# OwshenNetwork/owshen

Hardware: NVIDIA H100
Metric: groth16_withdraw_proofs_per_sec (higher is better)
Workload: dtype u256 (8x32-bit Montgomery limbs, integer)

## Files before the change

### bindings/rust/ffi.rs

```rust
#![allow(non_camel_case_types, dead_code)]
use std::os::raw::{c_char, c_void};

#[repr(C)] pub struct OgCtx { _private: [u8; 0] }
#[repr(C)] pub struct OgPk { _private: [u8; 0] }

pub const OG_OK: i32 = 0;
pub const OG_E_INVALID: i32 = -1;
pub const OG_E_ENCODING: i32 = -2;
pub const OG_E_NO_DEVICE: i32 = -3;
pub const OG_E_CUDA: i32 = -4;
pub const OG_E_NOMEM: i32 = -5;
pub const OG_E_VERIFY: i32 = -6;

extern "C" {
    pub fn og_abi_version() -> i32;
    pub fn og_strerror(code: i32) -> *const c_char;
    pub fn og_last_error(ctx: *const OgCtx) -> *const c_char;
    pub fn og_init(device: i32, out: *mut *mut OgCtx) -> i32;
    pub fn og_free(ctx: *mut OgCtx);
    pub fn og_sync(ctx: *mut OgCtx) -> i32;
    pub fn og_stream(ctx: *mut OgCtx, out_cuda_stream: *mut *mut c_void) -> i32;
    pub fn og_timer_start(ctx: *mut OgCtx) -> i32;
    pub fn og_timer_stop(ctx: *mut OgCtx, ms: *mut f32) -> i32;
    pub fn og_launch_count(ctx: *const OgCtx) -> u64;
// ... 91 lines not shown
    pub fn og_groth16_prove_labeled_association_dev(ctx: *mut OgCtx, pk: *const OgPk, d_tokens: *const u8, d_recipients: *const u8, d_withdrawn: *const u64, d_nullifiers: *const u8, d_secrets: *const u8, d_amounts: *const u64, d_labels: *const u32, d_siblings: *const u8, d_path_bits: *const u32, d_change_nullifiers: *const u8, d_change_secrets: *const u8, d_assoc_siblings: *const u8, d_assoc_path_bits: *const u32, batch: u32, d_rs: *const u8, d_proofs: *mut u8, d_public_out: *mut u8) -> i32;
    pub fn og_groth16_prove_owned_transfer(ctx: *mut OgCtx, pk: *const OgPk, roots: *const u8, tokens: *const u8, recipients: *const u8, in_spend_keys: *const u8, in_blindings: *const u8, in_amounts: *const u64, in_siblings: *const u8, in_path_bits: *const u32, out_owners: *const u8, out_blindings: *const u8, out_amounts: *const u64, batch: u32, rs: *const u8, proofs: *mut u8, public_out: *mut u8) -> i32;
    pub fn og_groth16_prove_owned_transfer_dev(ctx: *mut OgCtx, pk: *const OgPk, d_roots: *const u8, d_tokens: *const u8, d_recipients: *const u8, d_in_spend_keys: *const u8, d_in_blindings: *const u8, d_in_amounts: *const u64, d_in_siblings: *const u8, d_in_path_bits: *const u32, d_out_owners: *const u8, d_out_blindings: *const u8, d_out_amounts: *const u64, batch: u32, d_rs: *const u8, d_proofs: *mut u8, d_public_out: *mut u8) -> i32;
    pub fn og_groth16_h_evals(ctx: *mut OgCtx, pk: *const OgPk, witness: *const u8, out: *mut u8) -> i32;
    pub fn og_groth16_verify(vk: *const u8, vk_len: u64, public_inputs: *const u8, n_pub: u32, proof256: *const u8) -> i32;
    pub fn og_ptau_new(ctx: *mut OgCtx, log_max: u32, out: *mut u8, out_len: *mut u64) -> i32;
    pub fn og_ptau_contribute(ctx: *mut OgCtx, acc: *const u8, acc_len: u64, secrets96: *const u8, nonces96: *const u8, acc_out: *mut u8, acc_out_len: *mut u64, record_out: *mut u8, record_len: *mut u64) -> i32;
    pub fn og_ptau_verify(ctx: *mut OgCtx, prev: *const u8, prev_len: u64, next: *const u8, next_len: u64, record: *const u8, record_len: u64) -> i32;
    pub fn og_ptau_prepare(ctx: *mut OgCtx, acc: *const u8, acc_len: u64, n_constraints: u32, n_vars: u32, n_pub: u32, a_row_ptr: *const u32, a_col: *const u32, a_coeffs: *const u8, b_row_ptr: *const u32, b_col: *const u32, b_coeffs: *const u8, c_row_ptr: *const u32, c_col: *const u32, c_coeffs: *const u8, pk_out: *mut u8, pk_len: *mut u64, vk_out: *mut u8, vk_len: *mut u64) -> i32;
    pub fn og_ptau_prepare_withdraw(ctx: *mut OgCtx, acc: *const u8, acc_len: u64, depth: u32, pk_out: *mut u8, pk_len: *mut u64, vk_out: *mut u8, vk_len: *mut u64) -> i32;
    pub fn og_phase2_contribute(ctx: *mut OgCtx, pk: *const u8, pk_len: u64, vk: *const u8, vk_len: u64, delta32: *const u8, nonce32: *const u8, pk_out: *mut u8, pk_out_len: *mut u64, vk_out: *mut u8, vk_out_len: *mut u64, record_out: *mut u8, record_len: *mut u64) -> i32;
    pub fn og_phase2_verify(ctx: *mut OgCtx, pk_prev: *const u8, pk_prev_len: u64, vk_prev: *const u8, vk_prev_len: u64, pk_next: *const u8, pk_next_len: u64, vk_next: *const u8, vk_next_len: u64, record: *const u8, record_len: u64) -> i32;
    pub fn og_scale_points(ctx: *mut OgCtx, g2: i32, points: *const u8, scalars: *const u8, n: u64, per_point: i32, out: *mut u8) -> i32;
    pub fn og_intt_points(ctx: *mut OgCtx, g2: i32, points: *mut u8, log_m: u32) -> i32;
    pub fn og_msm_bucket_sums(ctx: *mut OgCtx, g2: i32, points: *const u8, n_points: u32, counts: *const u32, entries: *const u32, n_groups: u32, nb: u32, n_entries_max: u64, few_groups: i32, out_totals: *mut u8, out_buckets: *mut u8) -> i32;
    pub fn og_field_probe_raw(ctx: *mut OgCtx, unit: i32, op: i32, a: *const u8, b: *const u8, n: u64, out: *mut u8) -> i32;
}
```

### include/owshen_b200.h

```cpp
#ifndef OWSHEN_B200_H
#define OWSHEN_B200_H
#include <stdint.h>
#ifdef __cplusplus
extern "C" {
#endif

typedef struct og_ctx og_ctx;
typedef struct og_pk og_pk;

enum {
    OG_OK = 0,
    OG_E_INVALID = -1,
    OG_E_ENCODING = -2,
    OG_E_NO_DEVICE = -3,
    OG_E_CUDA = -4,
    OG_E_NOMEM = -5,
    OG_E_VERIFY = -6
};

int32_t og_abi_version(void);
const char* og_strerror(int32_t code);
const char* og_last_error(const og_ctx* ctx);

int32_t og_init(int32_t device, og_ctx** out);
// ... 260 lines not shown
int32_t og_ptau_prepare_withdraw(og_ctx* ctx, const uint8_t* acc, uint64_t acc_len, uint32_t depth, uint8_t* pk_out, uint64_t* pk_len,
                                 uint8_t* vk_out, uint64_t* vk_len);
int32_t og_phase2_contribute(og_ctx* ctx, const uint8_t* pk, uint64_t pk_len, const uint8_t* vk, uint64_t vk_len, const uint8_t* delta32,
                             const uint8_t* nonce32, uint8_t* pk_out, uint64_t* pk_out_len, uint8_t* vk_out, uint64_t* vk_out_len,
                             uint8_t* record_out, uint64_t* record_len);
int32_t og_phase2_verify(og_ctx* ctx, const uint8_t* pk_prev, uint64_t pk_prev_len, const uint8_t* vk_prev, uint64_t vk_prev_len,
                         const uint8_t* pk_next, uint64_t pk_next_len, const uint8_t* vk_next, uint64_t vk_next_len,
                         const uint8_t* record, uint64_t record_len);
int32_t og_scale_points(og_ctx* ctx, int32_t g2, const uint8_t* points, const uint8_t* scalars, uint64_t n, int32_t per_point,
                        uint8_t* out);
int32_t og_intt_points(og_ctx* ctx, int32_t g2, uint8_t* points, uint32_t log_m);

int32_t og_msm_bucket_sums(og_ctx* ctx, int32_t g2, const uint8_t* points, uint32_t n_points, const uint32_t* counts,
                           const uint32_t* entries, uint32_t n_groups, uint32_t nb, uint64_t n_entries_max, int32_t few_groups,
                           uint8_t* out_totals, uint8_t* out_buckets);
int32_t og_field_probe_raw(og_ctx* ctx, int32_t unit, int32_t op, const uint8_t* a, const uint8_t* b, uint64_t n, uint8_t* out);

#ifdef __cplusplus
}
#endif
#endif
```

### owshen_b200/api.py

```python
import array
import bisect
import ctypes as C
import os
import secrets as _rand
import subprocess

_HERE = os.path.dirname(os.path.abspath(__file__))
_LIB_PATH = os.environ.get("OWSHEN_B200_LIB") or os.path.join(_HERE, "libowshen_b200.so")
_lib = None

FR_MODULUS = 21888242871839275222246405745257275088548364400416034343698204186575808495617
PROOF_BYTES = 256

OG_OK, OG_E_INVALID, OG_E_VERIFY = 0, -1, -6

NOTE_SUBGROUP_ORDER = 2736030358979909402780800718157159386076813972158567259200215660948447373041
NOTE_NOT_OWNED, NOTE_MALFORMED = 0xFFFFFFFF, 0xFFFFFFFE
NOTE_RECORD_BYTES, NOTE_PLAINTEXT_BYTES = 160, 128


class OwshenB200Error(RuntimeError):
    def __init__(self, code, detail=""):
        self.code = code
        msg = lib().og_strerror(code).decode() if _lib is not None else str(code)
# ... 121 lines not shown
    "og_ptau_contribute": (C.c_int32, [C.c_void_p, C.c_void_p, C.c_uint64, C.c_void_p, C.c_void_p,
                                       C.c_void_p, C.POINTER(C.c_uint64), C.c_void_p, C.POINTER(C.c_uint64)]),
    "og_ptau_verify": (C.c_int32, [C.c_void_p, C.c_void_p, C.c_uint64, C.c_void_p, C.c_uint64, C.c_void_p, C.c_uint64]),
    "og_ptau_prepare": (C.c_int32, [C.c_void_p, C.c_void_p, C.c_uint64, C.c_uint32, C.c_uint32, C.c_uint32] + [C.c_void_p] * 9
                        + [C.c_void_p, C.POINTER(C.c_uint64), C.c_void_p, C.POINTER(C.c_uint64)]),
    "og_ptau_prepare_withdraw": (C.c_int32, [C.c_void_p, C.c_void_p, C.c_uint64, C.c_uint32,
                                             C.c_void_p, C.POINTER(C.c_uint64), C.c_void_p, C.POINTER(C.c_uint64)]),
    "og_phase2_contribute": (C.c_int32, [C.c_void_p, C.c_void_p, C.c_uint64, C.c_void_p, C.c_uint64, C.c_void_p, C.c_void_p,
                                         C.c_void_p, C.POINTER(C.c_uint64), C.c_void_p, C.POINTER(C.c_uint64),
                                         C.c_void_p, C.POINTER(C.c_uint64)]),
    "og_phase2_verify": (C.c_int32, [C.c_void_p] + [C.c_void_p, C.c_uint64] * 5),
    "og_scale_points": (C.c_int32, [C.c_void_p, C.c_int32, C.c_void_p, C.c_void_p, C.c_uint64, C.c_int32, C.c_void_p]),
    "og_intt_points": (C.c_int32, [C.c_void_p, C.c_int32, C.c_void_p, C.c_uint32]),
    "og_msm_bucket_sums": (C.c_int32, [C.c_void_p, C.c_int32, C.c_void_p, C.c_uint32, C.c_void_p, C.c_void_p, C.c_uint32, C.c_uint32,
                                       C.c_uint64, C.c_int32, C.c_void_p, C.c_void_p]),
    "og_field_probe_raw": (C.c_int32, [C.c_void_p, C.c_int32, C.c_int32, C.c_void_p, C.c_void_p, C.c_uint64, C.c_void_p]),
}
ABI_SYMBOLS = tuple(_SIGS)


def lib():
    global _lib
    if _lib is None:
        if not os.path.exists(_LIB_PATH):
            raise OSError(f"{_LIB_PATH} is missing: build it with owshen_b200.build_library() / "
                          "`make -C owshen_b200/csrc` -- there is no CPU fallback")
        L = C.CDLL(_LIB_PATH)
        for name, (res, args) in _SIGS.items():
            fn = getattr(L, name)
            fn.restype = res
# ... 227 lines not shown
            if not hasattr(xs, "astype"):
                return array.array("I", xs)
            a = array.array("I")
            a.frombytes(xs.astype("<u4").tobytes())
            return a
        cnt, ent = u32(counts), u32(entries)
        total = sum(cnt)
        _need(len(cnt) == n_groups * nb and len(ent) == total, "msm_bucket_sums: need n_groups * nb counts and sum(counts) entries")
        out = C.create_string_buffer(pb * n_groups)
        bk = C.create_string_buffer(pb * n_groups * nb) if buckets else None
        _check(lib().og_msm_bucket_sums(self._h, curve == "g2", points, len(points) // pb, C.c_void_p(cnt.buffer_info()[0]),
                                        C.c_void_p(ent.buffer_info()[0]) if total else None, n_groups, nb,
                                        total if n_entries_max is None else n_entries_max, int(few_groups), out, bk), self)
        return out.raw, (bk.raw if buckets else None)

    def mimc7_hash2(self, left: bytes, right: bytes) -> bytes:
        _need(len(left) % 32 == 0 and len(right) == len(left), "mimc7_hash2: left and right must be equally long multiples of 32 bytes")
        n = len(left) // 32
        out = C.create_string_buffer(32 * n)
        _check(lib().og_mimc7_hash2(self._h, left, right, n, out), self)
        return out.raw

    def merkle_paths(self, leaves: bytes, siblings: bytes, path_bits, depth: int) -> bytes:
        _need(0 <= depth <= 32 and len(leaves) % 32 == 0, "merkle_paths: depth must be <= 32 and leaves a multiple of 32 bytes")
        n = len(leaves) // 32
        _need(len(siblings) == 32 * n * depth and len(path_bits) == n, "merkle_paths: siblings must hold n*depth elements and path_bits n words")
        out = C.create_string_buffer(32 * n * (depth + 1))
        _check(lib().og_mimc7_merkle_paths(self._h, leaves, siblings, _bits_array(path_bits), n, depth, out), self)
        return out.raw

# ... 885 lines not shown
```

### owshen_b200/csrc/capi.cu

```cuda
#include <stdlib.h>
#include <new>
#include "common.cuh"
#include "groth16.cuh"
#include "mimc.cuh"
#include "msm.cuh"
#include "ntt.cuh"
#include "withdraw_circuit.hpp"

using namespace og;

void* og_ctx::slot(int id, size_t bytes) {
    if (bytes == 0) bytes = 32;
    if (slot_cap[id] >= bytes) return slot_ptr[id];
    cudaDeviceSynchronize();
    if (slot_ptr[id]) cudaFree(slot_ptr[id]);
    slot_ptr[id] = nullptr; slot_cap[id] = 0;
    size_t cap = bytes + bytes / 8;
    cudaError_t e = cudaMalloc(&slot_ptr[id], cap);
    if (e != cudaSuccess) {
        e = cudaMalloc(&slot_ptr[id], bytes);
        cap = bytes;
    }
    if (e != cudaSuccess) {
        snprintf(err, sizeof(err), "slot %d: cudaMalloc(%zu) failed: %s", id, bytes, cudaGetErrorString(e));
// ... 1457 lines not shown
    OG_SLOT(ctx, dtot, uint8_t, S_IO_E, pb * n_groups);
    uint8_t* dbk = nullptr;
    if (out_buckets) { dbk = (uint8_t*)ctx->slot(S_IO_F, pb * n_keys); if (!dbk) return OG_E_NOMEM; }
    OG_TRY(clear_flag(ctx));
    if (n_points) H2D(ctx, dp, points, pb * n_points);
    if (total) H2D(ctx, de, entries, 4 * total);
    H2D(ctx, dc, counts, 4ull * n_keys);
    H2D(ctx, doff, offsets.data(), 4ull * (n_keys + 1ull));
    if (g2) OG_TRY(msm_bucket_sums<Fq2>(ctx, dp, n_points, de, doff, dc, n_groups, nb, n_entries_max, few_groups != 0, dtot, dbk));
    else OG_TRY(msm_bucket_sums<Fq>(ctx, dp, n_points, de, doff, dc, n_groups, nb, n_entries_max, few_groups != 0, dtot, dbk));
    D2H(ctx, out_totals, dtot, pb * n_groups);
    if (out_buckets) D2H(ctx, out_buckets, dbk, pb * n_keys);
    return check_flag(ctx);
}

int32_t og_field_probe_raw(og_ctx* ctx, int32_t unit, int32_t op, const uint8_t* a, const uint8_t* b, uint64_t n, uint8_t* out) {
    OG_ENTER(ctx);
    const bool op_ok = unit ? (op >= 0 && op <= 7) : ((op >= 0 && op <= 3) || (op >= 8 && op <= 14));
    if (unit < 0 || unit > 1 || !op_ok || (n && (!a || !b || !out))) return OG_E_INVALID;
    if (n == 0) return OG_OK;
    const uint64_t eb = unit ? 64 : 32;
    OG_SLOT(ctx, da, uint8_t, S_IO_A, eb * n);
    OG_SLOT(ctx, db, uint8_t, S_IO_B, eb * n);
    OG_SLOT(ctx, dout, uint8_t, S_IO_C, eb * n);
    H2D(ctx, da, a, eb * n); H2D(ctx, db, b, eb * n);
    if (unit) OG_TRY(field_probe_raw<Fq2>(ctx, op, da, db, n, dout));
    else OG_TRY(field_probe_raw<Fq>(ctx, op, da, db, n, dout));
    D2H(ctx, out, dout, eb * n);
    OG_CUDA(ctx, cudaStreamSynchronize(ctx->stream));
    return OG_OK;
// ... 4 lines not shown
```

### owshen_b200/csrc/groth16.cu

```cuda
#include "groth16.cuh"
#include "mimc.cuh"
#include "msm.cuh"
#include "ntt.cuh"
#include "withdraw_circuit.hpp"
#include <stdlib.h>

namespace og {

__global__ void __launch_bounds__(128) k_extras(const uint8_t* __restrict__ rs, uint32_t batch, uint32_t n_vars, uint32_t w_stride,
                                                Fr* __restrict__ W, Fr* __restrict__ rs_m, int* flag) {
    uint32_t p = blockIdx.x * blockDim.x + threadIdx.x;
    if (p >= batch) return;
    Fr r = load_canonical<Fr>(rs + 64ull * p, flag);
    Fr s = load_canonical<Fr>(rs + 64ull * p + 32, flag);
    Fr* w = W + (size_t)p * w_stride;
    w[n_vars] = Fr::one();
    w[n_vars + 1] = r;
    rs_m[2 * p] = r;
    rs_m[2 * p + 1] = s;
}

__global__ void __launch_bounds__(128) k_witness_in(const uint8_t* __restrict__ in, uint32_t batch, uint32_t n_vars, uint32_t w_stride,
                                                    Fr* __restrict__ W, int* flag) {
    uint64_t t = (uint64_t)blockIdx.x * blockDim.x + threadIdx.x;
// ... 19 lines not shown
    if (j >= m) return;
    const Fr* w = W + (size_t)p * w_stride;
    Fr a = Fr::zero(), b = Fr::zero();
    if (j < n_constraints) {
        for (uint32_t k = A.row_ptr[j]; k < A.row_ptr[j + 1]; k++) a = a + A.val[k] * w[A.col[k]];
        for (uint32_t k = B.row_ptr[j]; k < B.row_ptr[j + 1]; k++) b = b + B.val[k] * w[B.col[k]];
    } else if (j <= n_constraints + n_pub) {
        a = w[j - n_constraints];
    }
    Fr* o = abc + (size_t)p * 3 * m;
    o[j] = a;
    o[m + j] = b;
    o[2 * m + j] = a * b;
}

__global__ void __launch_bounds__(128) k_pointwise(const Fr* __restrict__ abc, uint32_t log_m, uint32_t batch, Fr* __restrict__ csc,
                                                   uint32_t csc_stride, uint32_t off) {
    uint32_t m = 1u << log_m;
    uint32_t j = blockIdx.x * blockDim.x + threadIdx.x;
    uint32_t p = blockIdx.y;
    if (j >= m) return;
    const Fr* o = abc + (size_t)p * 3 * m;
    csc[(size_t)p * csc_stride + off + j] = o[j] * o[m + j] - o[2 * m + j];
}

__global__ void __launch_bounds__(128) k_compose(const Fr* __restrict__ W, uint32_t w_stride, const Fr* __restrict__ rs_m,
                                                 const uint32_t* __restrict__ supp, uint32_t n_supp, uint32_t n_vars, uint32_t n_pub,
                                                 uint32_t m, Fr* __restrict__ bsc, uint32_t bsc_stride, Fr* __restrict__ csc,
                                                 uint32_t csc_stride) {
    uint32_t t = blockIdx.x * blockDim.x + threadIdx.x;
    uint32_t p = blockIdx.y;
    const Fr* w = W + (size_t)p * w_stride;
    Fr* bs = bsc + (size_t)p * bsc_stride;
    Fr* cs = csc + (size_t)p * csc_stride;
    uint32_t n_priv = n_vars - n_pub - 1;
    Fr r = rs_m[2 * p], s = rs_m[2 * p + 1];
    if (t < n_priv) cs[t] = w[n_pub + 1 + t];
    if (t < n_supp) {
        Fr v = w[supp[t]];
        bs[t] = v;
        cs[n_priv + t] = r * v;
    }
    if (t == 0) {
        bs[n_supp] = Fr::one();
        bs[n_supp + 1] = s;
        cs[n_priv + n_supp + m] = r;
    }
}

__global__ void __launch_bounds__(32) k_assemble_g1(const G1XYZZ* __restrict__ totA, const G1XYZZ* __restrict__ totC,
                                                    const Fr* __restrict__ rs_m, uint32_t batch, uint8_t* __restrict__ proofs) {
    uint32_t p = blockIdx.x * blockDim.x + threadIdx.x;
    if (p >= batch) return;
    G1XYZZ a = totA[p];
    G1Affine A;
    xyzz_to_affine_ni(&A, &a);
    uint32_t s[8];
    rs_m[2 * p + 1].to_canonical(s);
    G1XYZZ acc = G1XYZZ::inf();
    for (int i = 255; i >= 0; i--) {
        xyzz_dbl_ni(&acc);
// ... 268 lines not shown
    b.sort_tiles = !s.tiles ? b.heavy : (uint32_t*)ctx->slot(S(S_PR_SORT_TILES, S_L1_SORT_TILES), s.tiles);
    if (!b.sort_stage || !b.sort_tiles) return OG_E_NOMEM;
    b.totC = b.totA + batch;
    b.totB = reinterpret_cast<G2XYZZ*>(b.totC + batch);
    return OG_OK;
}

template <class F>
static int32_t run_msm(og_ctx* ctx, const og_pk* pk, int which, ChunkBufs& b, uint32_t B, const Affine<F>* table, uint32_t n_pts,
                       const Fr* scalars, uint32_t stride, XYZZ<F>* totals) {
    DigitPlan plan;
    plan.scalars = reinterpret_cast<const uint32_t*>(scalars);
    plan.n = n_pts; plan.scalar_stride = stride; plan.n_problems = B;
    plan.c = pk->c[which]; plan.n_windows = pk->n_windows[which]; plan.nb = pk->nb[which];
    plan.key_stride_problem = 1; plan.key_stride_window = 0; plan.tidx_window_stride = n_pts;
    plan.montgomery = 1;
    uint32_t n_keys = B * pk->nb[which];
    OG_TRY(msm_sort_digits(ctx, plan, n_keys, b.counts, b.offsets, nullptr, b.sorted, b.sort_stage, b.sort_tiles));
    return msm_buckets(ctx, table, b.sorted, b.offsets, b.counts, B, pk->nb[which], (uint64_t)B * n_pts * pk->n_windows[which],
                       static_cast<XYZZ<F>*>(b.buckets), static_cast<XYZZ<F>*>(b.lvl), b.heavy, b.cursor, totals);
}

struct WitnessSource {
    const uint8_t* d_wit = nullptr;
    Statement stmt = ST_WITHDRAW;
    uint32_t depth = 0;
    StatementInputs in;
    uint8_t* d_public = nullptr;
};

static int32_t prove_chunk(og_ctx* ctx, const og_pk* pk, ChunkBufs& b, const WitnessSource& src, uint32_t off, uint32_t B,
// ... 112 lines not shown
    WitnessSource src;
    src.d_wit = d_wit;
    return prove_batch(ctx, pk, src, batch, d_rs, d_proofs);
}

int32_t h_evals_dev(og_ctx* ctx, const og_pk* pk, const uint8_t* d_wit, uint8_t* d_out) {
    ChunkBufs b;
    OG_TRY(alloc_chunk(ctx, pk, 1, 1, 0, b));
    const uint32_t m = 1u << pk->log_m, n_priv = pk->n_vars - pk->n_pub - 1;
    OG_LAUNCH(ctx, k_witness_in, (pk->n_vars + 127) / 128, 128, 0, d_wit, 1, pk->n_vars, b.w_stride, b.W, ctx->d_flag);
    CsrDev A{pk->a_ptr, pk->a_col, pk->a_val}, Bm{pk->b_ptr, pk->b_col, pk->b_val};
    OG_LAUNCH(ctx, k_abc, dim3((m + 127) / 128, 1), 128, 0, A, Bm, pk->n_constraints, pk->n_pub, pk->log_m, b.W, b.w_stride, 1, b.abc);
    OG_TRY(ntt_mont_dev(ctx, b.abc, b.ntt_tmp, pk->log_m, 3, 1, 0, 1));
    OG_TRY(ntt_mont_dev(ctx, b.abc, b.ntt_tmp, pk->log_m, 3, 0, 1, 2));
    OG_LAUNCH(ctx, k_pointwise, dim3((m + 127) / 128, 1), 128, 0, b.abc, pk->log_m, 1, b.csc, b.csc_stride, n_priv + pk->n_supp);
    return mimc_from_mont_dev(ctx, b.csc + n_priv + pk->n_supp, m, d_out);
}

int32_t statement_witness_bytes_dev(og_ctx* ctx, Statement s, uint32_t depth, const StatementInputs& in, uint32_t batch, uint8_t* d_out) {
    const uint32_t nv = STATEMENTS[s].shape(depth).n_vars;
    Fr* W = (Fr*)ctx->slot(S_PR_WIT, sizeof(Fr) * (size_t)batch * nv);
    if (!W) return OG_E_NOMEM;
    OG_TRY(statement_witness_dev(ctx, s, depth, nv, in, batch, W));
    uint64_t tot = (uint64_t)batch * nv;
    OG_LAUNCH(ctx, k_witness_out, (unsigned)((tot + 127) / 128), 128, 0, W, batch, nv, nv, d_out);
    return OG_OK;
}

}
```

### owshen_b200/csrc/msm.cu

```cuda
#ifdef OG_MSM_G1
#define OG_FQ_SQR_CALL
#endif
#include "msm.cuh"
#include "glv.cuh"
#include <stdlib.h>
#if !defined(OG_MSM_G1) && !defined(OG_MSM_G2)
#error "compile msm.cu with -DOG_MSM_G1 or -DOG_MSM_G2"
#endif

namespace og {

template <class F> struct FieldIO;
template <> struct FieldIO<Fq> {
    static constexpr int BYTES = 32;
    static __device__ __forceinline__ Fq load(const uint8_t* p, int* flag) { return load_canonical<Fq>(p, flag); }
    static __device__ __forceinline__ void store(uint8_t* p, const Fq& v) { store_canonical(p, v); }
};
template <> struct FieldIO<Fq2> {
    static constexpr int BYTES = 64;
    static __device__ __forceinline__ Fq2 load(const uint8_t* p, int* flag) {
        return Fq2{load_canonical<Fq>(p, flag), load_canonical<Fq>(p + 32, flag)};
    }
    static __device__ __forceinline__ void store(uint8_t* p, const Fq2& v) { store_canonical(p, v.c0); store_canonical(p + 32, v.c1); }
};
// ... 167 lines not shown
        run += c[k];
    }
}

static int32_t exclusive_scan(og_ctx* ctx, const uint32_t* d_counts, uint32_t n, uint32_t* d_offsets, uint32_t* d_cursor) {
    uint32_t n_tiles = (n + SCAN_TILE - 1) / SCAN_TILE;
    OG_SLOT(ctx, tile_sums, uint32_t, ctx->lane ? S_L1_MSM_MISC : S_MSM_MISC, 4 * (size_t)n_tiles);
    OG_LAUNCH(ctx, k_scan_tiles, n_tiles, SCAN_THREADS, 0, d_counts, n, tile_sums);
    OG_LAUNCH(ctx, k_scan_tile_sums, 1, SCAN_THREADS, 0, tile_sums, n_tiles, d_offsets + n);
    OG_LAUNCH(ctx, k_scan_apply, n_tiles, SCAN_THREADS, 0, d_counts, n, tile_sums, d_offsets, d_cursor);
    return OG_OK;
}

constexpr uint32_t SORT_PARTS = 128, SORT_TILE = 4096, SORT_THREADS = 256;
constexpr uint32_t SORT_MAX_NB = 32768, SORT_MAX_FINE = SORT_MAX_NB / SORT_PARTS;
constexpr uint32_t NO_BIN = 0xFFFFFFFFu;
static_assert(SORT_THREADS == SCAN_THREADS, "k_sort_local scans with block_exclusive_scan");
static_assert(SORT_PARTS <= SORT_THREADS && SORT_MAX_FINE <= SORT_THREADS && SORT_TILE % SORT_THREADS == 0, "sort shape");
static_assert(SORT_MAX_FINE <= 256, "fine bucket ids are staged as one byte");

static uint32_t sort_parts(uint32_t nb) { return nb < SORT_PARTS ? nb : SORT_PARTS; }
static uint32_t sort_shift(uint32_t nb) { uint32_t s = 0; while ((sort_parts(nb) << s) < nb) s++; return s; }
static uint64_t sort_tiles(uint64_t n) { return (n + SORT_TILE - 1) / SORT_TILE; }

__device__ __forceinline__ uint32_t warp_bin_add(uint32_t* bins, uint32_t bin) {
    const uint32_t lane = threadIdx.x & 31, valid = __ballot_sync(0xffffffffu, bin != NO_BIN);
    if (!valid) return 0;
    const uint32_t leader = __ffs(valid) - 1, first = __shfl_sync(0xffffffffu, bin, leader);
    if (__all_sync(0xffffffffu, bin == NO_BIN || bin == first)) {
        uint32_t base = 0;
        if (lane == leader) base = atomicAdd(&bins[first], (uint32_t)__popc(valid));
        return __shfl_sync(0xffffffffu, base, leader) + __popc(valid & ((1u << lane) - 1));
    }
    return bin != NO_BIN ? atomicAdd(&bins[bin], 1u) : 0;
}

__global__ void __launch_bounds__(SORT_THREADS) k_sort_part_count(DigitPlan P, uint32_t shift, uint32_t n_tiles,
                                                                  uint32_t* __restrict__ tile_counts, int* flag) {
    __shared__ uint32_t hist[SORT_PARTS];
    const uint32_t prob = blockIdx.y, tile = blockIdx.x, parts = P.nb >> shift;
    for (uint32_t p = threadIdx.x; p < parts; p += SORT_THREADS) hist[p] = 0;
    __syncthreads();
    const uint64_t lo = (uint64_t)tile * SORT_TILE, hi = lo + SORT_TILE < P.n ? lo + SORT_TILE : P.n;
    uint32_t raw[8];
    if (lo + threadIdx.x < hi) DigitIter::fetch(P, prob, lo + threadIdx.x, raw);
    for (uint64_t i0 = lo; i0 < hi; i0 += SORT_THREADS) {
        const uint64_t i = i0 + threadIdx.x;
        DigitIter it;
        if (!(i < hi && it.from_raw(P, raw, flag))) it.clear();
        if (i + SORT_THREADS < hi) DigitIter::fetch(P, prob, i + SORT_THREADS, raw);
        it.windows(P, [&](uint32_t, uint32_t mag, uint32_t) { warp_bin_add(hist, mag ? (mag - 1) >> shift : NO_BIN); });
    }
    __syncthreads();
    for (uint32_t p = threadIdx.x; p < parts; p += SORT_THREADS) tile_counts[((size_t)prob * parts + p) * n_tiles + tile] = hist[p];
}

constexpr uint32_t SORT_ROUND_WINDOWS = 24, SORT_ROUND = SORT_THREADS * SORT_ROUND_WINDOWS;
__global__ void __launch_bounds__(SORT_THREADS) k_sort_part_scatter(DigitPlan P, uint32_t shift, uint32_t n_tiles,
                                                                    const uint32_t* __restrict__ tile_offs, uint32_t* __restrict__ stage_e,
                                                                    uint8_t* __restrict__ stage_f, int* flag) {
    __shared__ uint32_t sm_e[SORT_ROUND];
    __shared__ uint16_t sm_b[SORT_ROUND];
    __shared__ uint32_t cnt[SORT_PARTS], lbase[SORT_PARTS], cur[SORT_PARTS];
    const uint32_t tid = threadIdx.x, prob = blockIdx.y, tile = blockIdx.x, parts = P.nb >> shift, fmask = (1u << shift) - 1;
    for (uint32_t p = tid; p < parts; p += SORT_THREADS) { cur[p] = tile_offs[((size_t)prob * parts + p) * n_tiles + tile]; cnt[p] = 0; }
    __syncthreads();
    const uint64_t lo = (uint64_t)tile * SORT_TILE, hi = lo + SORT_TILE < P.n ? lo + SORT_TILE : P.n;
    uint32_t raw[8];
    if (lo + tid < hi) DigitIter::fetch(P, prob, lo + tid, raw);
    for (uint64_t i0 = lo; i0 < hi; i0 += SORT_THREADS) {
        const uint64_t i = i0 + tid;
        DigitIter it;
        if (!(i < hi && it.from_raw(P, raw, flag))) it.clear();
        if (i + SORT_THREADS < hi) DigitIter::fetch(P, prob, i + SORT_THREADS, raw);
        for (uint32_t w0 = 0; w0 < P.n_windows; w0 += SORT_ROUND_WINDOWS) {
            auto bin_of = [&](uint32_t w, uint32_t mag) { return mag && w >= w0 && w < w0 + SORT_ROUND_WINDOWS ? (mag - 1) >> shift : NO_BIN; };
            it.windows(P, [&](uint32_t w, uint32_t mag, uint32_t) { warp_bin_add(cnt, bin_of(w, mag)); });
            __syncthreads();
            uint32_t n_round, b = block_exclusive_scan(tid < parts ? cnt[tid] : 0, &n_round);
            if (tid < parts) { lbase[tid] = b; cnt[tid] = b; }
            __syncthreads();
            it.windows(P, [&](uint32_t w, uint32_t mag, uint32_t neg) {
                const uint32_t bin = bin_of(w, mag), pos = warp_bin_add(cnt, bin);
                if (bin != NO_BIN) { sm_e[pos] = (((uint32_t)i + w * P.tidx_window_stride) << 1) | neg; sm_b[pos] = (uint16_t)(mag - 1); }
            });
            __syncthreads();
            for (uint32_t k = tid; k < n_round; k += SORT_THREADS) {
                const uint32_t bk = sm_b[k], p = bk >> shift, dst = cur[p] + k - lbase[p];
                stage_e[dst] = sm_e[k];
                stage_f[dst] = (uint8_t)(bk & fmask);
            }
            __syncthreads();
            if (tid < parts) { cur[tid] += cnt[tid] - lbase[tid]; cnt[tid] = 0; }
            __syncthreads();
        }
    }
}

constexpr uint32_t SORT_LOCAL_CAP = 10240;
constexpr uint32_t SORT_LOCAL_ITEMS = 8, SORT_LOCAL_STEP = SORT_THREADS * SORT_LOCAL_ITEMS;
__global__ void __launch_bounds__(SORT_THREADS) k_sort_local(const uint32_t* __restrict__ tile_offs, uint32_t n_tiles, uint32_t n_parts,
                                                             uint32_t shift, const uint32_t* __restrict__ total,
                                                             const uint32_t* __restrict__ stage_e, const uint8_t* __restrict__ stage_f,
                                                             uint32_t* __restrict__ counts, uint32_t* __restrict__ offsets,
                                                             uint32_t* __restrict__ sorted) {
    __shared__ uint32_t bins[SORT_THREADS];
    __shared__ uint32_t sm_out[SORT_LOCAL_CAP];
    const uint32_t g = blockIdx.x, F = 1u << shift, tid = threadIdx.x;
// ... 29 lines not shown
#pragma unroll
        for (uint32_t k = 0; k < SORT_LOCAL_ITEMS; k++) {
            const uint32_t pos = warp_bin_add(bins, f[k]);
            if (f[k] != NO_BIN) { if (staged) sm_out[pos - start] = e[k]; else sorted[pos] = e[k]; }
        }
    }
    if (staged) {
        __syncthreads();
        for (uint32_t k = tid; k < end - start; k += SORT_THREADS) sorted[start + k] = sm_out[k];
    }
}

size_t msm_sort_stage_bytes(uint64_t n_entries) { return 5 * n_entries; }
size_t msm_sort_tile_bytes(uint32_t n_problems, uint32_t nb, uint64_t n) { return 8 * (size_t)n_problems * sort_parts(nb) * sort_tiles(n) + 4; }

int32_t msm_sort_digits(og_ctx* ctx, const DigitPlan& plan, uint32_t n_keys, uint32_t* d_counts, uint32_t* d_offsets,
                        uint32_t* d_cursor, uint32_t* d_sorted, uint32_t* d_stage, uint32_t* d_tiles) {
    if (plan.n == 0 || plan.n_problems == 0) {
        OG_CUDA(ctx, cudaMemsetAsync(d_counts, 0, sizeof(uint32_t) * (size_t)n_keys, ctx->stream));
        OG_CUDA(ctx, cudaMemsetAsync(d_offsets, 0, sizeof(uint32_t) * ((size_t)n_keys + 1), ctx->stream));
        return OG_OK;
    }
    if (plan.key_stride_window == 0) {
        if (!d_stage || !d_tiles || plan.key_stride_problem != 1 || plan.nb > SORT_MAX_NB || n_keys != plan.n_problems * plan.nb) return OG_E_INVALID;
        const uint32_t parts = sort_parts(plan.nb), shift = sort_shift(plan.nb), n_tiles = (uint32_t)sort_tiles(plan.n);
        const uint32_t n_parts = plan.n_problems * parts, n_runs = n_parts * n_tiles;
        uint32_t* tile_counts = d_tiles;
        uint32_t* tile_offs = d_tiles + n_runs;
        uint32_t* stage_e = d_stage;
        uint8_t* stage_f = reinterpret_cast<uint8_t*>(d_stage + (uint64_t)plan.n_problems * plan.n * plan.n_windows);
        dim3 tgrid(n_tiles, plan.n_problems);
        OG_LAUNCH(ctx, k_sort_part_count, tgrid, SORT_THREADS, 0, plan, shift, n_tiles, tile_counts, ctx->d_flag);
        OG_TRY(exclusive_scan(ctx, tile_counts, n_runs, tile_offs, nullptr));
        OG_LAUNCH(ctx, k_sort_part_scatter, tgrid, SORT_THREADS, 0, plan, shift, n_tiles, tile_offs, stage_e, stage_f, ctx->d_flag);
        OG_LAUNCH(ctx, k_sort_local, n_parts, SORT_THREADS, 0, tile_offs, n_tiles, n_parts, shift, tile_offs + n_runs, stage_e, stage_f,
                  d_counts, d_offsets, d_sorted);
        return OG_OK;
    }
    OG_CUDA(ctx, cudaMemsetAsync(d_counts, 0, sizeof(uint32_t) * (size_t)n_keys, ctx->stream));
    dim3 grid((unsigned)((plan.n + 255) / 256), plan.n_problems);
    OG_LAUNCHN(ctx, "k_digits_count", k_digits<false>, grid, 256, 0, plan, d_counts, nullptr, nullptr, nullptr, ctx->d_flag);
    OG_TRY(exclusive_scan(ctx, d_counts, n_keys, d_offsets, d_cursor));
    OG_LAUNCHN(ctx, "k_digits_scatter", k_digits<true>, grid, 256, 0, plan, d_counts, d_offsets, d_cursor, d_sorted, ctx->d_flag);
    return OG_OK;
}
#endif


constexpr uint32_t ORDER_BINS = 2048;
template <class F>
__global__ void __launch_bounds__(1024) k_bucket_order(const uint32_t* __restrict__ counts, uint32_t nb, uint32_t* __restrict__ perm) {
    __shared__ uint32_t hist[ORDER_BINS];
// ... 837 lines not shown
```

Before: 2131.

## Template MSM digit sort on window size and keep scalars canonical

Specializes the partitioned MSM digit-sort kernels on the window width C, so window count, part count and shift become compile-time constants and the digit loops are fully unrolled. The scatter kernel now packs bucket, sign, window and scalar index into one 32-bit shared slot and can process two scalars per thread per round, cutting shared-memory traffic and the number of block-wide syncs. Groth16 witness and H scalars are written in canonical form at composition and pointwise time, so the B/C MSM sorts skip the Montgomery conversion and the final from-Montgomery pass becomes a plain copy. Instantiating 15 template variants increases code size, and the packed slot format limits windows to 128 and rounds to 512 scalars. A new sort_digits API entry point is also added.

```diff
diff --git a/bindings/rust/ffi.rs b/bindings/rust/ffi.rs
--- a/bindings/rust/ffi.rs
+++ b/bindings/rust/ffi.rs
@@ -129,5 +129,6 @@
     pub fn og_scale_points(ctx: *mut OgCtx, g2: i32, points: *const u8, scalars: *const u8, n: u64, per_point: i32, out: *mut u8) -> i32;
     pub fn og_intt_points(ctx: *mut OgCtx, g2: i32, points: *mut u8, log_m: u32) -> i32;
     pub fn og_msm_bucket_sums(ctx: *mut OgCtx, g2: i32, points: *const u8, n_points: u32, counts: *const u32, entries: *const u32, n_groups: u32, nb: u32, n_entries_max: u64, few_groups: i32, out_totals: *mut u8, out_buckets: *mut u8) -> i32;
+    pub fn og_msm_sort_digits(ctx: *mut OgCtx, scalars: *const u8, n: u64, n_problems: u32, c: u32, montgomery: i32, out_counts: *mut u32, out_offsets: *mut u32, out_sorted: *mut u32) -> i32;
     pub fn og_field_probe_raw(ctx: *mut OgCtx, unit: i32, op: i32, a: *const u8, b: *const u8, n: u64, out: *mut u8) -> i32;
 }
diff --git a/include/owshen_b200.h b/include/owshen_b200.h
--- a/include/owshen_b200.h
+++ b/include/owshen_b200.h
@@ -298,6 +298,8 @@
 int32_t og_msm_bucket_sums(og_ctx* ctx, int32_t g2, const uint8_t* points, uint32_t n_points, const uint32_t* counts,
                            const uint32_t* entries, uint32_t n_groups, uint32_t nb, uint64_t n_entries_max, int32_t few_groups,
                            uint8_t* out_totals, uint8_t* out_buckets);
+int32_t og_msm_sort_digits(og_ctx* ctx, const uint8_t* scalars, uint64_t n, uint32_t n_problems, uint32_t c, int32_t montgomery,
+                           uint32_t* out_counts, uint32_t* out_offsets, uint32_t* out_sorted);
 int32_t og_field_probe_raw(og_ctx* ctx, int32_t unit, int32_t op, const uint8_t* a, const uint8_t* b, uint64_t n, uint8_t* out);
 
 #ifdef __cplusplus
diff --git a/owshen_b200/api.py b/owshen_b200/api.py
--- a/owshen_b200/api.py
+++ b/owshen_b200/api.py
@@ -159,6 +159,8 @@
     "og_intt_points": (C.c_int32, [C.c_void_p, C.c_int32, C.c_void_p, C.c_uint32]),
     "og_msm_bucket_sums": (C.c_int32, [C.c_void_p, C.c_int32, C.c_void_p, C.c_uint32, C.c_void_p, C.c_void_p, C.c_uint32, C.c_uint32,
                                        C.c_uint64, C.c_int32, C.c_void_p, C.c_void_p]),
+    "og_msm_sort_digits": (C.c_int32, [C.c_void_p, C.c_void_p, C.c_uint64, C.c_uint32, C.c_uint32, C.c_int32, C.c_void_p, C.c_void_p,
+                                       C.c_void_p]),
     "og_field_probe_raw": (C.c_int32, [C.c_void_p, C.c_int32, C.c_int32, C.c_void_p, C.c_void_p, C.c_uint64, C.c_void_p]),
 }
 ABI_SYMBOLS = tuple(_SIGS)
@@ -416,6 +418,15 @@
                                         total if n_entries_max is None else n_entries_max, int(few_groups), out, bk), self)
         return out.raw, (bk.raw if buckets else None)
 
+    def msm_sort_digits(self, scalars: bytes, n: int, n_problems: int, c: int, montgomery=False):
+        _need(len(scalars) == 32 * n * n_problems, "msm_sort_digits: need 32 * n * n_problems bytes of scalars")
+        _need(2 <= c <= 16, "msm_sort_digits: c must lie in [2, 16]")
+        n_keys, n_ent = n_problems << (c - 1), n * n_problems * ((255 + c - 1) // c)
+        cnt, off, srt = array.array("I", bytes(4 * n_keys)), array.array("I", bytes(4 * (n_keys + 1))), array.array("I", bytes(4 * n_ent))
+        _check(lib().og_msm_sort_digits(self._h, scalars, n, n_problems, c, int(montgomery), C.c_void_p(cnt.buffer_info()[0]),
+                                        C.c_void_p(off.buffer_info()[0]), C.c_void_p(srt.buffer_info()[0])), self)
+        return cnt.tolist(), off.tolist(), srt[:off[n_keys]].tolist()
+
     def mimc7_hash2(self, left: bytes, right: bytes) -> bytes:
         _need(len(left) % 32 == 0 and len(right) == len(left), "mimc7_hash2: left and right must be equally long multiples of 32 bytes")
         n = len(left) // 32
diff --git a/owshen_b200/csrc/capi.cu b/owshen_b200/csrc/capi.cu
--- a/owshen_b200/csrc/capi.cu
+++ b/owshen_b200/csrc/capi.cu
@@ -1495,6 +1495,44 @@
     return check_flag(ctx);
 }
 
+int32_t og_msm_sort_digits(og_ctx* ctx, const uint8_t* scalars, uint64_t n, uint32_t n_problems, uint32_t c, int32_t montgomery,
+                           uint32_t* out_counts, uint32_t* out_offsets, uint32_t* out_sorted) {
+    OG_ENTER(ctx);
+    if (!scalars || !out_counts || !out_offsets || !out_sorted || montgomery < 0 || montgomery > 1) return OG_E_INVALID;
+    const uint32_t W = c >= 2 && c <= 16 ? msm_windows(c) : 0;
+    if (!W || n == 0 || n_problems == 0 || n_problems > 65535 || n * W >= (1ull << 31) || n * W * n_problems > 0xFFFFFFFFull ||
+        ((uint64_t)n_problems << (c - 1)) > (1ull << 26)) {
+        snprintf(ctx->err, sizeof(ctx->err), "c must lie in [2, 16], n_problems in [1, 65535], n * windows < 2^31, all entries < 2^32, "
+                 "n_problems * 2^(c-1) <= 2^26");
+        return OG_E_INVALID;
+    }
+    const uint32_t nb = 1u << (c - 1), n_keys = n_problems * nb;
+    const uint64_t n_sc = n * n_problems, n_ent = n_sc * W;
+    OG_SLOT(ctx, dsc, uint8_t, S_IO_A, 32 * n_sc);
+    OG_SLOT(ctx, dc, uint32_t, S_IO_B, 4ull * n_keys);
+    OG_SLOT(ctx, doff, uint32_t, S_IO_C, 4ull * (n_keys + 1ull));
+    OG_SLOT(ctx, dsorted, uint32_t, S_IO_D, 4 * n_ent);
+    OG_SLOT(ctx, dstage, uint32_t, S_IO_E, msm_sort_stage_bytes(n_ent));
+    OG_SLOT(ctx, dtiles, uint32_t, S_IO_F, msm_sort_tile_bytes(n_problems, nb, n));
+    OG_SLOT(ctx, dmont, Fr, S_IO_G, montgomery ? 32 * n_sc : 32);
+    OG_TRY(clear_flag(ctx));
+    H2D(ctx, dsc, scalars, 32 * n_sc);
+    if (montgomery) OG_TRY(mimc_to_mont_dev(ctx, dsc, n_sc, dmont));
+    DigitPlan plan;
+    plan.scalars = montgomery ? reinterpret_cast<const uint32_t*>(dmont) : reinterpret_cast<const uint32_t*>(dsc);
+    plan.n = n; plan.scalar_stride = n; plan.n_problems = n_problems;
+    plan.c = c; plan.n_windows = W; plan.nb = nb;
+    plan.key_stride_problem = 1; plan.key_stride_window = 0; plan.tidx_window_stride = (uint32_t)n;
+    plan.montgomery = montgomery;
+    OG_TRY(msm_sort_digits(ctx, plan, n_keys, dc, doff, nullptr, dsorted, dstage, dtiles));
+    OG_TRY(check_flag(ctx));
+    D2H(ctx, out_counts, dc, 4ull * n_keys);
+    D2H(ctx, out_offsets, doff, 4ull * (n_keys + 1ull));
+    OG_CUDA(ctx, cudaStreamSynchronize(ctx->stream));
+    if (out_offsets[n_keys]) D2H(ctx, out_sorted, dsorted, 4ull * out_offsets[n_keys]);
+    return check_flag(ctx);
+}
+
 int32_t og_field_probe_raw(og_ctx* ctx, int32_t unit, int32_t op, const uint8_t* a, const uint8_t* b, uint64_t n, uint8_t* out) {
     OG_ENTER(ctx);
     const bool op_ok = unit ? (op >= 0 && op <= 7) : ((op >= 0 && op <= 3) || (op >= 8 && op <= 14));
diff --git a/owshen_b200/csrc/groth16.cu b/owshen_b200/csrc/groth16.cu
--- a/owshen_b200/csrc/groth16.cu
+++ b/owshen_b200/csrc/groth16.cu
@@ -57,6 +57,8 @@
     o[2 * m + j] = a * b;
 }
 
+static __device__ __forceinline__ Fr canonical(const Fr& v) { Fr o; v.to_canonical(o.l); return o; }
+
 __global__ void __launch_bounds__(128) k_pointwise(const Fr* __restrict__ abc, uint32_t log_m, uint32_t batch, Fr* __restrict__ csc,
                                                    uint32_t csc_stride, uint32_t off) {
     uint32_t m = 1u << log_m;
@@ -64,7 +66,7 @@
     uint32_t p = blockIdx.y;
     if (j >= m) return;
     const Fr* o = abc + (size_t)p * 3 * m;
-    csc[(size_t)p * csc_stride + off + j] = o[j] * o[m + j] - o[2 * m + j];
+    csc[(size_t)p * csc_stride + off + j] = canonical(o[j] * o[m + j] - o[2 * m + j]);
 }
 
 __global__ void __launch_bounds__(128) k_compose(const Fr* __restrict__ W, uint32_t w_stride, const Fr* __restrict__ rs_m,
@@ -78,16 +80,16 @@
     Fr* cs = csc + (size_t)p * csc_stride;
     uint32_t n_priv = n_vars - n_pub - 1;
     Fr r = rs_m[2 * p], s = rs_m[2 * p + 1];
-    if (t < n_priv) cs[t] = w[n_pub + 1 + t];
+    if (t < n_priv) cs[t] = canonical(w[n_pub + 1 + t]);
     if (t < n_supp) {
         Fr v = w[supp[t]];
-        bs[t] = v;
-        cs[n_priv + t] = r * v;
+        bs[t] = canonical(v);
+        cs[n_priv + t] = canonical(r * v);
     }
     if (t == 0) {
-        bs[n_supp] = Fr::one();
-        bs[n_supp + 1] = s;
-        cs[n_priv + n_supp + m] = r;
+        bs[n_supp] = canonical(Fr::one());
+        bs[n_supp + 1] = canonical(s);
+        cs[n_priv + n_supp + m] = canonical(r);
     }
 }
 
@@ -386,7 +388,7 @@
     plan.n = n_pts; plan.scalar_stride = stride; plan.n_problems = B;
     plan.c = pk->c[which]; plan.n_windows = pk->n_windows[which]; plan.nb = pk->nb[which];
     plan.key_stride_problem = 1; plan.key_stride_window = 0; plan.tidx_window_stride = n_pts;
-    plan.montgomery = 1;
+    plan.montgomery = which == 0;
     uint32_t n_keys = B * pk->nb[which];
     OG_TRY(msm_sort_digits(ctx, plan, n_keys, b.counts, b.offsets, nullptr, b.sorted, b.sort_stage, b.sort_tiles));
     return msm_buckets(ctx, table, b.sorted, b.offsets, b.counts, B, pk->nb[which], (uint64_t)B * n_pts * pk->n_windows[which],
@@ -529,7 +531,8 @@
     OG_TRY(ntt_mont_dev(ctx, b.abc, b.ntt_tmp, pk->log_m, 3, 1, 0, 1));
     OG_TRY(ntt_mont_dev(ctx, b.abc, b.ntt_tmp, pk->log_m, 3, 0, 1, 2));
     OG_LAUNCH(ctx, k_pointwise, dim3((m + 127) / 128, 1), 128, 0, b.abc, pk->log_m, 1, b.csc, b.csc_stride, n_priv + pk->n_supp);
-    return mimc_from_mont_dev(ctx, b.csc + n_priv + pk->n_supp, m, d_out);
+    OG_CUDA(ctx, cudaMemcpyAsync(d_out, b.csc + n_priv + pk->n_supp, 32ull * m, cudaMemcpyDeviceToDevice, ctx->stream));
+    return OG_OK;
 }
 
 int32_t statement_witness_bytes_dev(og_ctx* ctx, Statement s, uint32_t depth, const StatementInputs& in, uint32_t batch, uint8_t* d_out) {
diff --git a/owshen_b200/csrc/msm.cu b/owshen_b200/csrc/msm.cu
--- a/owshen_b200/csrc/msm.cu
+++ b/owshen_b200/csrc/msm.cu
@@ -205,14 +205,28 @@
 
 constexpr uint32_t SORT_PARTS = 128, SORT_TILE = 4096, SORT_THREADS = 256;
 constexpr uint32_t SORT_MAX_NB = 32768, SORT_MAX_FINE = SORT_MAX_NB / SORT_PARTS;
+constexpr uint32_t SORT_MIN_C = 2, SORT_MAX_C = 16;
 constexpr uint32_t NO_BIN = 0xFFFFFFFFu;
 static_assert(SORT_THREADS == SCAN_THREADS, "k_sort_local scans with block_exclusive_scan");
 static_assert(SORT_PARTS <= SORT_THREADS && SORT_MAX_FINE <= SORT_THREADS && SORT_TILE % SORT_THREADS == 0, "sort shape");
 static_assert(SORT_MAX_FINE <= 256, "fine bucket ids are staged as one byte");
 
 static uint32_t sort_parts(uint32_t nb) { return nb < SORT_PARTS ? nb : SORT_PARTS; }
-static uint32_t sort_shift(uint32_t nb) { uint32_t s = 0; while ((sort_parts(nb) << s) < nb) s++; return s; }
 static uint64_t sort_tiles(uint64_t n) { return (n + SORT_TILE - 1) / SORT_TILE; }
+
+template <uint32_t C> struct SortShape {
+    static_assert(C >= SORT_MIN_C && C <= SORT_MAX_C, "window bits");
+    static constexpr uint32_t NW = (255 + C - 1) / C;
+    static constexpr uint32_t NB = 1u << (C - 1);
+    static constexpr uint32_t PARTS = NB < SORT_PARTS ? NB : SORT_PARTS;
+    static constexpr uint32_t SHIFT = C - 1 > 7 ? C - 1 - 7 : 0;
+    static __device__ __forceinline__ uint32_t digit(const uint32_t s[9], uint32_t w, uint32_t& carry) {
+        const uint32_t bit = w * C, word = bit >> 5;
+        const uint32_t v = (__funnelshift_r(s[word], s[word + 1], bit & 31) & ((1u << C) - 1)) + carry;
+        carry = v > (1u << (C - 1));
+        return carry ? ((1u << C) - v) | 0x10000u : v;
+    }
+};
 
 __device__ __forceinline__ uint32_t warp_bin_add(uint32_t* bins, uint32_t bin) {
     const uint32_t lane = threadIdx.x & 31, valid = __ballot_sync(0xffffffffu, bin != NO_BIN);
@@ -226,11 +240,12 @@
     return bin != NO_BIN ? atomicAdd(&bins[bin], 1u) : 0;
 }
 
-__global__ void __launch_bounds__(SORT_THREADS) k_sort_part_count(DigitPlan P, uint32_t shift, uint32_t n_tiles,
-                                                                  uint32_t* __restrict__ tile_counts, int* flag) {
-    __shared__ uint32_t hist[SORT_PARTS];
-    const uint32_t prob = blockIdx.y, tile = blockIdx.x, parts = P.nb >> shift;
-    for (uint32_t p = threadIdx.x; p < parts; p += SORT_THREADS) hist[p] = 0;
+template <uint32_t C>
+__global__ void __launch_bounds__(SORT_THREADS) k_sort_part_count(DigitPlan P, uint32_t n_tiles, uint32_t* __restrict__ tile_counts, int* flag) {
+    using S = SortShape<C>;
+    __shared__ uint32_t hist[S::PARTS];
+    const uint32_t prob = blockIdx.y, tile = blockIdx.x;
+    if (threadIdx.x < S::PARTS) hist[threadIdx.x] = 0;
     __syncthreads();
     const uint64_t lo = (uint64_t)tile * SORT_TILE, hi = lo + SORT_TILE < P.n ? lo + SORT_TILE : P.n;
     uint32_t raw[8];
@@ -240,49 +255,85 @@
         DigitIter it;
         if (!(i < hi && it.from_raw(P, raw, flag))) it.clear();
         if (i + SORT_THREADS < hi) DigitIter::fetch(P, prob, i + SORT_THREADS, raw);
-        it.windows(P, [&](uint32_t, uint32_t mag, uint32_t) { warp_bin_add(hist, mag ? (mag - 1) >> shift : NO_BIN); });
-    }
-    __syncthreads();
-    for (uint32_t p = threadIdx.x; p < parts; p += SORT_THREADS) tile_counts[((size_t)prob * parts + p) * n_tiles + tile] = hist[p];
-}
-
-constexpr uint32_t SORT_ROUND_WINDOWS = 24, SORT_ROUND = SORT_THREADS * SORT_ROUND_WINDOWS;
-__global__ void __launch_bounds__(SORT_THREADS) k_sort_part_scatter(DigitPlan P, uint32_t shift, uint32_t n_tiles,
-                                                                    const uint32_t* __restrict__ tile_offs, uint32_t* __restrict__ stage_e,
-                                                                    uint8_t* __restrict__ stage_f, int* flag) {
-    __shared__ uint32_t sm_e[SORT_ROUND];
-    __shared__ uint16_t sm_b[SORT_ROUND];
-    __shared__ uint32_t cnt[SORT_PARTS], lbase[SORT_PARTS], cur[SORT_PARTS];
-    const uint32_t tid = threadIdx.x, prob = blockIdx.y, tile = blockIdx.x, parts = P.nb >> shift, fmask = (1u << shift) - 1;
-    for (uint32_t p = tid; p < parts; p += SORT_THREADS) { cur[p] = tile_offs[((size_t)prob * parts + p) * n_tiles + tile]; cnt[p] = 0; }
+        uint32_t carry = 0;
+#pragma unroll
+        for (uint32_t w = 0; w < S::NW; w++) {
+            const uint32_t mag = S::digit(it.s, w, carry) & 0xFFFFu;
+            warp_bin_add(hist, mag ? (mag - 1) >> S::SHIFT : NO_BIN);
+        }
+    }
+    __syncthreads();
+    if (threadIdx.x < S::PARTS) tile_counts[((size_t)prob * S::PARTS + threadIdx.x) * n_tiles + tile] = hist[threadIdx.x];
+}
+
+constexpr uint32_t SORT_ROUND_SLOTS = SORT_THREADS * 34;
+template <uint32_t C>
+__global__ void __launch_bounds__(SORT_THREADS) k_sort_part_scatter(DigitPlan P, uint32_t n_tiles, const uint32_t* __restrict__ tile_offs,
+                                                                    uint32_t* __restrict__ stage_e, uint8_t* __restrict__ stage_f, int* flag) {
+    using S = SortShape<C>;
+    constexpr uint32_t WPT = SORT_ROUND_SLOTS / SORT_THREADS;
+    constexpr uint32_t SPT = 2 * S::NW <= WPT ? 2 : 1;
+    constexpr uint32_t RW = SPT == 2 || S::NW <= WPT ? S::NW : WPT, NR = (S::NW + RW - 1) / RW;
+    constexpr uint32_t ROUND = SPT * SORT_THREADS, FMASK = (1u << S::SHIFT) - 1;
+    static_assert(S::NW <= 128 && ROUND <= 512 && SORT_TILE % ROUND == 0, "slot = bucket << 17 | negative << 16 | window << 9 | scalar");
+    __shared__ uint32_t sm[SPT * RW * SORT_THREADS];
+    __shared__ uint32_t cnt[S::PARTS], dst0[S::PARTS];
+    const uint32_t tid = threadIdx.x, prob = blockIdx.y, tile = blockIdx.x;
+    uint32_t cur = 0;
+    if (tid < S::PARTS) { cur = tile_offs[((size_t)prob * S::PARTS + tid) * n_tiles + tile]; cnt[tid] = 0; }
     __syncthreads();
     const uint64_t lo = (uint64_t)tile * SORT_TILE, hi = lo + SORT_TILE < P.n ? lo + SORT_TILE : P.n;
-    uint32_t raw[8];
-    if (lo + tid < hi) DigitIter::fetch(P, prob, lo + tid, raw);
-    for (uint64_t i0 = lo; i0 < hi; i0 += SORT_THREADS) {
-        const uint64_t i = i0 + tid;
-        DigitIter it;
-        if (!(i < hi && it.from_raw(P, raw, flag))) it.clear();
-        if (i + SORT_THREADS < hi) DigitIter::fetch(P, prob, i + SORT_THREADS, raw);
-        for (uint32_t w0 = 0; w0 < P.n_windows; w0 += SORT_ROUND_WINDOWS) {
-            auto bin_of = [&](uint32_t w, uint32_t mag) { return mag && w >= w0 && w < w0 + SORT_ROUND_WINDOWS ? (mag - 1) >> shift : NO_BIN; };
-            it.windows(P, [&](uint32_t w, uint32_t mag, uint32_t) { warp_bin_add(cnt, bin_of(w, mag)); });
-            __syncthreads();
-            uint32_t n_round, b = block_exclusive_scan(tid < parts ? cnt[tid] : 0, &n_round);
-            if (tid < parts) { lbase[tid] = b; cnt[tid] = b; }
-            __syncthreads();
-            it.windows(P, [&](uint32_t w, uint32_t mag, uint32_t neg) {
-                const uint32_t bin = bin_of(w, mag), pos = warp_bin_add(cnt, bin);
-                if (bin != NO_BIN) { sm_e[pos] = (((uint32_t)i + w * P.tidx_window_stride) << 1) | neg; sm_b[pos] = (uint16_t)(mag - 1); }
-            });
-            __syncthreads();
-            for (uint32_t k = tid; k < n_round; k += SORT_THREADS) {
-                const uint32_t bk = sm_b[k], p = bk >> shift, dst = cur[p] + k - lbase[p];
-                stage_e[dst] = sm_e[k];
-                stage_f[dst] = (uint8_t)(bk & fmask);
+    uint32_t raw[SPT][8];
+#pragma unroll
+    for (uint32_t j = 0; j < SPT; j++)
+        if (lo + j * SORT_THREADS + tid < hi) DigitIter::fetch(P, prob, lo + j * SORT_THREADS + tid, raw[j]);
+    for (uint64_t i0 = lo; i0 < hi; i0 += ROUND) {
+        DigitIter it[SPT];
+        uint32_t carry[SPT];
+#pragma unroll
+        for (uint32_t j = 0; j < SPT; j++) {
+            const uint64_t i = i0 + j * SORT_THREADS + tid;
+            if (!(i < hi && it[j].from_raw(P, raw[j], flag))) it[j].clear();
+            if (i + ROUND < hi) DigitIter::fetch(P, prob, i + ROUND, raw[j]);
+            carry[j] = 0;
+        }
+#pragma unroll
+        for (uint32_t r = 0; r < NR; r++) {
+#pragma unroll
+            for (uint32_t j = 0; j < SPT; j++) {
+                uint32_t cr = carry[j];
+#pragma unroll
+                for (uint32_t k = 0; k < RW; k++) {
+                    const uint32_t w = r * RW + k;
+                    uint32_t bin = NO_BIN;
+                    if (w < S::NW) { const uint32_t mag = S::digit(it[j].s, w, cr) & 0xFFFFu; if (mag) bin = (mag - 1) >> S::SHIFT; }
+                    warp_bin_add(cnt, bin);
+                }
             }
             __syncthreads();
-            if (tid < parts) { cur[tid] += cnt[tid] - lbase[tid]; cnt[tid] = 0; }
+            const uint32_t c = tid < S::PARTS ? cnt[tid] : 0;
+            uint32_t n_round;
+            const uint32_t base = block_exclusive_scan(c, &n_round);
+            if (tid < S::PARTS) { cnt[tid] = base; dst0[tid] = cur - base; cur += c; }
+            __syncthreads();
+#pragma unroll
+            for (uint32_t j = 0; j < SPT; j++) {
+#pragma unroll
+                for (uint32_t k = 0; k < RW; k++) {
+                    const uint32_t w = r * RW + k;
+                    uint32_t bin = NO_BIN, dg = 0;
+                    if (w < S::NW) { dg = S::digit(it[j].s, w, carry[j]); const uint32_t mag = dg & 0xFFFFu; if (mag) bin = (mag - 1) >> S::SHIFT; }
+                    const uint32_t pos = warp_bin_add(cnt, bin);
+                    if (bin != NO_BIN) sm[pos] = ((dg & 0xFFFFu) - 1) << 17 | (dg >> 16) << 16 | w << 9 | (j * SORT_THREADS + tid);
+                }
+            }
+            __syncthreads();
+            if (tid < S::PARTS) cnt[tid] = 0;
+            for (uint32_t k = tid; k < n_round; k += SORT_THREADS) {
+                const uint32_t v = sm[k], bk = v >> 17, dst = dst0[bk >> S::SHIFT] + k;
+                stage_e[dst] = (((uint32_t)i0 + (v & 511u) + ((v >> 9) & 127u) * P.tidx_window_stride) << 1) | ((v >> 16) & 1u);
+                stage_f[dst] = (uint8_t)(bk & FMASK);
+            }
             __syncthreads();
         }
     }
@@ -342,6 +393,31 @@
 size_t msm_sort_stage_bytes(uint64_t n_entries) { return 5 * n_entries; }
 size_t msm_sort_tile_bytes(uint32_t n_problems, uint32_t nb, uint64_t n) { return 8 * (size_t)n_problems * sort_parts(nb) * sort_tiles(n) + 4; }
 
+template <uint32_t C>
+static int32_t sort_partitioned(og_ctx* ctx, const DigitPlan& plan, uint32_t* d_counts, uint32_t* d_offsets, uint32_t* d_sorted,
+                                uint32_t* d_stage, uint32_t* d_tiles) {
+    using S = SortShape<C>;
+    const uint32_t n_tiles = (uint32_t)sort_tiles(plan.n), n_parts = plan.n_problems * S::PARTS, n_runs = n_parts * n_tiles;
+    uint32_t* tile_counts = d_tiles;
+    uint32_t* tile_offs = d_tiles + n_runs;
+    uint32_t* stage_e = d_stage;
+    uint8_t* stage_f = reinterpret_cast<uint8_t*>(d_stage + (uint64_t)plan.n_problems * plan.n * S::NW);
+    dim3 tgrid(n_tiles, plan.n_problems);
+    OG_LAUNCHN(ctx, "k_sort_part_count", k_sort_part_count<C>, tgrid, SORT_THREADS, 0, plan, n_tiles, tile_counts, ctx->d_flag);
+    OG_TRY(exclusive_scan(ctx, tile_counts, n_runs, tile_offs, nullptr));
+    OG_LAUNCHN(ctx, "k_sort_part_scatter", k_sort_part_scatter<C>, tgrid, SORT_THREADS, 0, plan, n_tiles, tile_offs, stage_e, stage_f, ctx->d_flag);
+    OG_LAUNCH(ctx, k_sort_local, n_parts, SORT_THREADS, 0, tile_offs, n_tiles, n_parts, S::SHIFT, tile_offs + n_runs, stage_e, stage_f,
+              d_counts, d_offsets, d_sorted);
+    return OG_OK;
+}
+template <uint32_t C>
+static int32_t sort_partitioned_c(og_ctx* ctx, const DigitPlan& plan, uint32_t* d_counts, uint32_t* d_offsets, uint32_t* d_sorted,
+                                  uint32_t* d_stage, uint32_t* d_tiles) {
+    if (plan.c == C) return sort_partitioned<C>(ctx, plan, d_counts, d_offsets, d_sorted, d_stage, d_tiles);
+    if constexpr (C < SORT_MAX_C) return sort_partitioned_c<C + 1>(ctx, plan, d_counts, d_offsets, d_sorted, d_stage, d_tiles);
+    return OG_E_INVALID;
+}
+
 int32_t msm_sort_digits(og_ctx* ctx, const DigitPlan& plan, uint32_t n_keys, uint32_t* d_counts, uint32_t* d_offsets,
                         uint32_t* d_cursor, uint32_t* d_sorted, uint32_t* d_stage, uint32_t* d_tiles) {
     if (plan.n == 0 || plan.n_problems == 0) {
@@ -350,20 +426,10 @@
         return OG_OK;
     }
     if (plan.key_stride_window == 0) {
-        if (!d_stage || !d_tiles || plan.key_stride_problem != 1 || plan.nb > SORT_MAX_NB || n_keys != plan.n_problems * plan.nb) return OG_E_INVALID;
-        const uint32_t parts = sort_parts(plan.nb), shift = sort_shift(plan.nb), n_tiles = (uint32_t)sort_tiles(plan.n);
-        const uint32_t n_parts = plan.n_problems * parts, n_runs = n_parts * n_tiles;
-        uint32_t* tile_counts = d_tiles;
-        uint32_t* tile_offs = d_tiles + n_runs;
-        uint32_t* stage_e = d_stage;
-        uint8_t* stage_f = reinterpret_cast<uint8_t*>(d_stage + (uint64_t)plan.n_problems * plan.n * plan.n_windows);
-        dim3 tgrid(n_tiles, plan.n_problems);
-        OG_LAUNCH(ctx, k_sort_part_count, tgrid, SORT_THREADS, 0, plan, shift, n_tiles, tile_counts, ctx->d_flag);
-        OG_TRY(exclusive_scan(ctx, tile_counts, n_runs, tile_offs, nullptr));
-        OG_LAUNCH(ctx, k_sort_part_scatter, tgrid, SORT_THREADS, 0, plan, shift, n_tiles, tile_offs, stage_e, stage_f, ctx->d_flag);
-        OG_LAUNCH(ctx, k_sort_local, n_parts, SORT_THREADS, 0, tile_offs, n_tiles, n_parts, shift, tile_offs + n_runs, stage_e, stage_f,
-                  d_counts, d_offsets, d_sorted);
-        return OG_OK;
+        if (!d_stage || !d_tiles || plan.key_stride_problem != 1 || plan.c < SORT_MIN_C || plan.c > SORT_MAX_C || plan.nb != 1u << (plan.c - 1) ||
+            plan.n_windows != msm_windows(plan.c) || n_keys != plan.n_problems * plan.nb)
+            return OG_E_INVALID;
+        return sort_partitioned_c<SORT_MIN_C>(ctx, plan, d_counts, d_offsets, d_sorted, d_stage, d_tiles);
     }
     OG_CUDA(ctx, cudaMemsetAsync(d_counts, 0, sizeof(uint32_t) * (size_t)n_keys, ctx->stream));
     dim3 grid((unsigned)((plan.n + 255) / 256), plan.n_problems);
```

Measured after the change: 2176 (median of 6 runs). 1.02x the previous value.
